# JGI-Bioinformatics/Kmernator

Hardware: AMD Instinct MI355X
Metric: total k-mers/sec at k=31, 150 bp reads (spectrum build, inputs resident in HBM) (higher is better)
Workload: dtype u64

## Files before the change

### kmernator_amd/csrc/kmr_api.hip

```cpp
#include <hip/hip_runtime.h>
#include <dlfcn.h>
#include <unistd.h>
#include <rccl/rccl.h>

#include <algorithm>
#include <atomic>
#include <cmath>
#include <cstdio>
#include <cstdlib>
#include <cstring>
#include <cctype>
#include <memory>
#include <string>
#include <type_traits>
#include <vector>

#include "../../include/kmernator_amd.h"
#include "kmr_kernels.hpp"
#include "kmr_partition.hpp"
#include "kmr_ingest.hpp"
#include "kmr_artifact.hpp"
#include "kmr_select.hpp"
#include "kmr_pairs.hpp"
#include "kmr_dump.hpp"
// ... 117 lines not shown
	uint64_t target_list = 2048;
	uint64_t sub_batch_bases = 0;
	int recycle = -1;
	int part_blocks = 0;
	double entry_share = -1.0;
	double early_entry_share = -1.0;
	uint64_t saturated_batch_bytes = 0;
	bool no_lut = false, no_narrow = false, no_l1_state = false, no_stream_lookups = false;
	uint64_t long_list_chunks = 0;
	uint64_t binned_min = 1ull << 18;
	uint64_t twobit_piece_bases = 0;
	uint64_t list_aim = 0;
	bool pow2_lists = false;
	bool no_packed_direct = false;
	bool no_uniform_count = false;
	bool no_lean_extract = false;
	bool exchange_fail_once = false;
	uint64_t dump_piece_bytes = 0;
	bool dump_timing = false;
	bool select_timing = false;
	bool pairs_timing = false;
	uint32_t pair_hash_bits = 64;
	bool no_coarse_lists = true;
};

struct kmr_handle : HandleMem, BuildMem, ExchangeMem {
	kmr_config cfg;
	Tuning tune;
	uint32_t k = 0, kb = 0, hkb = 0, W = 0;
	bool ext = false;
// ... 16 lines not shown
	long trk_next = 128; uint64_t trk_raw = 0, trk_good = 0; std::vector<unsigned long long> trk_bounds; std::vector<uint64_t> trk_snap_raw, trk_snap_good;
	bool sk_fast_div = false;
	bool sender_launch = false;
	bool sk_exchange = false;
	bool auto_mode = false;
	int bits1 = 0;
	uint64_t inserted_records = 0;
	uint64_t call_bases_hint = 0;
	uint32_t lut_log2 = 0;
	uint64_t lut_gen = ~0ull, map_gen = 0;
	hipStream_t tb_copy_stream = nullptr; hipEvent_t tb_ready[2] = {nullptr, nullptr}, tb_consumed[2] = {nullptr, nullptr}; bool tb_set_used[2] = {false, false};
	const SkPacked *packed_direct = nullptr;
	int uniform_q_hint = -1;
	uint32_t sk_bits = 0, sk_m = 0, sk_off = 0, sk_win = 0;
	double hP[256], hPk[256];
	uint32_t sk_uni_w = 0xffffffffu; bool sk_uni_mixed = false; bool last_count_uniform = false;
	uint32_t peer_uni_w = 0xffffffffu; bool peer_uni_mixed = false, peers_declare = false;
	uint64_t xr_lo = 0, xr_hi = ~0ull;
	uint64_t last_early_hi = 0, last_early_entries = 0;
	bool last_early_overflowed = false;
	double last_score_ms = 0, last_select_ms = 0, last_write_ms = 0;
	double last_dump_size_ms = 0, last_dump_write_ms = 0;
	double last_pairs_ms = 0, last_pairs_parse_ms = 0, last_pairs_sort_ms = 0;
	uint64_t last_pair_hash_collisions = 0;
	uint64_t last_saturated_keys = 0, last_saturated_batches = 0;
	bool qual_mixed = false;
	uint32_t sk_fine_shift = 0;
	uint32_t sk_min_override = 0;
	uint64_t xo_segcap = 0; std::vector<uint64_t> xo_counts; const void *xo_batch = nullptr; uint64_t xo_first = 0;
	void *xc_comm = nullptr; kmr_transport xc_tr = {nullptr, nullptr, nullptr};
	uint64_t xc_job_bases = 0, xc_bytes_to_peers = 0;
// ... 1435 lines not shown
		if (dv[1]) mixed = true;
		else if (dv[0] != SK_UNI_NONE) { if (w == SK_UNI_NONE) w = dv[0]; else if (w != dv[0]) mixed = true; }
	}
	if (!mixed && w != SK_UNI_NONE) { uni = true; uni_wbits = w; }
	return 0;
}
template <int W> SkLong<W> sk_own_lists(kmr_handle *h, bool refined) {
	SkLong<W> lg{};
	lg.list_first = 0; lg.list_stride = 1;
	if (h->sk_exchange && h->cfg.world_size > 1 && !refined) { lg.list_first = h->cfg.rank; lg.list_stride = h->cfg.world_size; }
	return lg;
}
template <int W> struct SkCountLaunch {
	void (*kern)(PoolView, const uint64_t *, const uint64_t *, uint64_t, uint32_t, CountOut, FinalizeParams, unsigned int *, uint32_t, SkTrackView, SkLong<W>);
	size_t smem;
};
template <int W, int LOG2S, bool TRACK, bool EXT, bool UNI> SkCountLaunch<W> sk_count_form() { return {sk_count_kernel<W, LOG2S, TRACK, EXT, UNI>, sk_count_smem_bytes<W, LOG2S, TRACK, EXT, UNI>()}; }
template <int W> int sk_count_select(kmr_handle *h, bool ext, bool tracking, bool uni, SkCountLaunch<W> &k) {
	k = ext ? sk_count_form<W, COUNT_LOG2S_EXT, false, true, false>() : (tracking ? sk_count_form<W, COUNT_LOG2S, true, false, false>() :
	    (uni ? sk_count_form<W, COUNT_LOG2S, false, false, true>() : sk_count_form<W, COUNT_LOG2S, false, false, false>()));
	const auto kern = k.kern; const size_t smem = k.smem;
	HIPCHK(h, hipFuncSetAttribute((const void *)kern, hipFuncAttributeMaxDynamicSharedMemorySize, (int)smem));
	return 0;
}

template <int W> struct SkFinalize {
	FinalizeParams f{}; bool keepSing = false, ext = false, tracking = false, refined = false, uni = false;
	uint64_t nl = 1; uint64_t *ls = nullptr, *lc = nullptr; uint32_t nch = 0;
	uint64_t wcap = 0, scap = 0, wmax = 0, smax = 0;
	uint32_t *wc = nullptr, *sc = nullptr; FinalizeCounters *fc = nullptr; unsigned long long *cursors = nullptr;
	SkTrackView tv{};
	SkLong<W> lgMain{}, lgItems{}; uint64_t n_items = 0;
	uint64_t early_slots = 0; FinalizeCounters early_c{};
	FinalizeCounters c{}; unsigned long long cur[2] = {0, 0};
};
// ... 123 lines not shown
		if (ext && (key_entries(h, h->uw_keys) < wcap || !h->uw_vals)) {
			h->uw_keys.reset(); h->uw_vals.reset();
			HIPCHK(h, h->uw_keys.alloc(8ull * W * wcap)); HIPCHK(h, h->uw_vals.alloc(4ull * vw * wcap));
		}
		if (key_entries(h, h->us_keys) < scap || !h->us_b8 || (ext && !h->us_pkt)) {
			h->us_keys.reset(); h->us_b8.reset(); h->us_pkt.reset();
			HIPCHK(h, h->us_keys.alloc(8ull * W * scap)); HIPCHK(h, h->us_b8.alloc(scap)); if (ext) HIPCHK(h, h->us_pkt.alloc(4 * scap));
		}
		HIPCHK(h, hipMemsetAsync(wc, 0, 4 * h->nb_weak, h->stream)); HIPCHK(h, hipMemsetAsync(sc, 0, 4 * h->nb_sing, h->stream));
		HIPCHK(h, hipMemsetAsync(fc, 0, sizeof(FinalizeCounters), h->stream)); HIPCHK(h, hipMemsetAsync(cursors, 0, 16, h->stream));
		const CountOut out = count_out(h, !ext, cursors, wc, sc, fc);
		rc = zero_work_counter(h); if (rc) return rc;
		const int grid = (int)std::min<uint64_t>((uint64_t)num_cus(h) * 4, (nl / p.lgMain.list_stride + SK_LBATCH) / SK_LBATCH);
		SkCountLaunch<W> k;
		rc = sk_count_select<W>(h, ext, tracking, p.uni, k); if (rc) return rc;
		if (tracking) HIPCHK(h, hipMemsetAsync(tv.d_unique, 0, 8 * (tv.n + 1), h->stream));
		if (dbg()) { int nb = 0; hipOccupancyMaxActiveBlocksPerMultiprocessor(&nb, (const void *)k.kern, SKC_THREADS, k.smem); fprintf(stderr, "sk_count<W=%d>: %d blocks per CU (LDS %zu), %llu lists, %u chunks\n", W, nb, k.smem, (unsigned long long)nl, p.nch); }
		hipLaunchKernelGGL(k.kern, dim3(grid), dim3(SKC_THREADS), k.smem, h->stream, pool_view(h, h->l1), p.ls, p.lc, nl, h->k, out, f, h->work_counter.get<unsigned int>(), sk_dbg_flags("KMR_SK_COUNT_DBG"), tv, p.lgMain);
		HIPCHK(h, hipGetLastError());
		DevBuf mslots, mext;
		if (n_items) {
			SkLong<W> &lgItems = p.lgItems;
			if (mslots.alloc(sizeof(Slot<W>) << merge_log2) != hipSuccess) return fail(h, KMR_ERR_OOM, "merge table of the long lists");
			if (ext && mext.alloc(sizeof(ExtSlot) << merge_log2) != hipSuccess) return fail(h, KMR_ERR_OOM, "merge table of the long lists");
			hipLaunchKernelGGL(table_clear_kernel<W>, dim3(grid_for(1ull << merge_log2)), dim3(256), 0, h->stream, mslots.get<Slot<W>>(), mext.get<ExtSlot>(), 1ull << merge_log2);
			lgItems.merge.slots = mslots.get<Slot<W>>(); lgItems.merge.ext = mext.get<ExtSlot>(); lgItems.merge.log2cap = merge_log2;
			HIPCHK(h, hipMemsetAsync(lgItems.merge_used, 0, 8, h->stream));
			rc = zero_work_counter(h); if (rc) return rc;
			const int grid2 = (int)std::min<uint64_t>((uint64_t)num_cus(h) * 4, n_items);
			hipLaunchKernelGGL(k.kern, dim3(grid2), dim3(SKC_THREADS), k.smem, h->stream, pool_view(h, h->l1), p.ls, p.lc, nl, h->k, out, f, h->work_counter.get<unsigned int>(), sk_dbg_flags("KMR_SK_COUNT_DBG"), tv, lgItems);
// ... 46 lines not shown
	p.keepSing = p.f.has_singletons && min_depth <= 1;
	p.ext = h->ext;
	p.tracking = h->cfg.size_tracker != 0;
	if (!h->l1.head) { rc = pool_reserve(h, h->l1, 0, false); if (rc) return rc; }
	rc = arena_reset(h); if (rc) return rc;
	p.nl = h->sk_state ? sk_list_count(h->sk_bits) : 1;
	if (h->sk_state) {
		hipLaunchKernelGGL(sk_close_kernel, dim3(grid_for(p.nl)), dim3(256), 0, h->stream, h->sk_state.get<unsigned long long>(), p.nl, h->l1.chunk_count.get<uint32_t>(), h->l1.cap);
		HIPCHK(h, hipGetLastError());
	}
	p.refined = h->sk_state && h->sk_fine_shift > 0;
	if (p.refined) { rc = sk_refine_lists(h, p.nl); if (rc) return rc; }
	rc = build_csr(h, h->l1, p.nl, 0, &p.ls, &p.lc, &p.nch); if (rc) return rc;
	rc = sk_entry_buffers<W>(h, p, h->stats.raw_good_kmers); if (rc) return rc;
	rc = sk_count_uniform<W>(h, p.tracking, p.uni, p.f.uni_wbits); if (rc) return rc;
	h->last_count_uniform = p.uni;
	if (p.tracking) { rc = sk_track_view(h, p.tv); if (rc) return rc; }
	p.lgMain = sk_own_lists<W>(h, p.refined);
	bool device_error = false;
	rc = sk_early_takeover<W>(h, p, min_depth, device_error); if (rc) return rc;
	if (device_error) { time_end(h, 1, ea, eb); return sync_state(h); }
	rc = sk_long_items<W>(h, p); if (rc) return rc;
	bool overflowed = false;
	rc = sk_count_pass<W>(h, p, overflowed); if (rc) return rc;
	if (overflowed) { time_end(h, 1, ea, eb); return fail(h, KMR_ERR_CAPACITY, "entry buffers of the count pass overflowed at their upper bound (internal sizing error)"); }
	h->stats.unique_kmers = p.c.unique;
	h->stats.singleton_kmers = p.f.has_singletons ? p.c.singletons : 0;
	if (p.tracking) { rc = sk_track_elements(h, p.tv, p.f.has_singletons); if (rc) return rc; }
	if (p.early_slots) { rc = sk_append_early<W>(h, p); if (rc) return rc; }
	h->early.active = false;
	hipEvent_t tma, tmb; time_begin(h, KMR_TIME_BUCKETS, &tma, &tmb);
// ... 238 lines not shown
int kmr_tune(kmr_handle *h, const char *knob, double value) {
	if (!h || !knob) return KMR_ERR_INVALID_ARG;
	const std::string k(knob);
	if (k == "target_list_records") h->tune.target_list = value >= 1 ? (uint64_t)value : 2048;
	else if (k == "sub_batch_bases") h->tune.sub_batch_bases = value >= 1 ? (uint64_t)value : 0;
	else if (k == "recycle_chunks") h->tune.recycle = value < 0 ? -1 : (value != 0 ? 1 : 0);
	else if (k == "partition_blocks") h->tune.part_blocks = value >= 1 ? (int)value : 0;
	else if (k == "entry_share") h->tune.entry_share = value;
	else if (k == "early_entry_share") h->tune.early_entry_share = value;
	else if (k == "saturated_batch_bytes") h->tune.saturated_batch_bytes = value >= 1 ? (uint64_t)value : 0;
	else if (k == "lookup_table") h->tune.no_lut = value == 0;
	else if (k == "stream_lookups") h->tune.no_stream_lookups = value == 0;
	else if (k == "long_list_chunks") h->tune.long_list_chunks = value < 2 ? 2 : (uint64_t)value;
	else if (k == "lean_extract") h->tune.no_lean_extract = value == 0;
	else if (k == "uniform_count") h->tune.no_uniform_count = value == 0;
	else if (k == "packed_direct") h->tune.no_packed_direct = value == 0;
	else if (k == "pow2_lists") h->tune.pow2_lists = value != 0;
	else if (k == "list_aim") h->tune.list_aim = value >= 1 ? (uint64_t)value : 0;
	else if (k == "twobit_piece_bases") h->tune.twobit_piece_bases = (uint64_t)value;
	else if (k == "exchange_fail_once") h->tune.exchange_fail_once = value != 0;
	else if (k == "binned_buckets_min") h->tune.binned_min = value >= 0 ? (uint64_t)value : ~0ull;
	else if (k == "coarse_lists") h->tune.no_coarse_lists = value == 0;
	else if (k == "select_timing") h->tune.select_timing = value != 0;
	else if (k == "dump_timing") h->tune.dump_timing = value != 0;
	else if (k == "pairs_timing") h->tune.pairs_timing = value != 0;
	else if (k == "pair_hash_bits") h->tune.pair_hash_bits = value >= 1 && value < 64 ? (uint32_t)value : 64;
	else if (k == "dump_piece_bytes") h->tune.dump_piece_bytes = value >= 1 ? (uint64_t)value : 0;
	else if (k == "narrow_tallies") h->tune.no_narrow = value == 0;
	else if (k == "keep_level1_state") h->tune.no_l1_state = value == 0;
	else if (k == "superkmer_window") {
		if (h->superkmer_mode && !h->sk_state) { uint32_t w, m, o; if (!sk_geometry(h->k, 0, w, m, o, (uint32_t)value)) return fail(h, KMR_ERR_INVALID_ARG, "no minimizer geometry under that window"); h->sk_win = w; h->sk_m = m; h->sk_off = o; }
	}
	else if (k == "superkmer_minimizer") {
		if (h->superkmer_mode && !h->sk_state) { uint32_t w, m, o; if (!sk_geometry(h->k, (uint32_t)value, w, m, o)) return fail(h, KMR_ERR_INVALID_ARG, "no minimizer geometry for that length"); h->sk_win = w; h->sk_m = m; h->sk_off = o; }
	}
	else return fail(h, KMR_ERR_INVALID_ARG, "unknown tuning knob '" + k + "'");
	return KMR_OK;
}

int kmr_build_info(kmr_handle *h, const char *what, double *value) {
	if (!h || !what || !value) return KMR_ERR_INVALID_ARG;
	const std::string k(what);
	if (k == "lists") *value = h->sk_state ? (double)sk_list_count(h->sk_bits) : 0.0;
	else if (k == "uniform_count") *value = h->last_count_uniform ? 1.0 : 0.0;
	else if (k == "chunk_pool_chunks") *value = (double)h->l1.cap;
	else if (k == "superkmer_window") *value = (double)h->sk_win;
	else if (k == "early_lists") *value = (double)h->last_early_hi;
	else if (k == "early_entries") *value = (double)h->last_early_entries;
	else if (k == "early_overflowed") *value = h->last_early_overflowed ? 1.0 : 0.0;
	else if (k == "saturated_keys") *value = (double)h->last_saturated_keys;
	else if (k == "saturated_batches") *value = (double)h->last_saturated_batches;
	else if (k == "device_blocks_live") *value = (double)g_blocks_live.load();
	else if (k == "filter_score_ms") *value = h->last_score_ms;
	else if (k == "select_ms") *value = h->last_select_ms;
	else if (k == "select_write_ms") *value = h->last_write_ms;
	else if (k == "pairs_ms") *value = h->last_pairs_ms;
	else if (k == "pairs_parse_ms") *value = h->last_pairs_parse_ms;
	else if (k == "pairs_sort_ms") *value = h->last_pairs_sort_ms;
	else if (k == "pair_hash_collisions") *value = (double)h->last_pair_hash_collisions;
// ... 1804 lines not shown
```

### kmernator_amd/csrc/kmr_instances.hpp

```cpp
#ifndef KMR_INSTANCES_HPP_
#define KMR_INSTANCES_HPP_

#include "kmr_superkmer.hpp"

namespace kmr {

static const int COUNT_LOG2S = 10;
static const int COUNT_LOG2S_EXT = 9;
static const int PD_THREADS = 1024, PD_RPT = 8, PD_LINE = 4;

#ifdef KMR_INSTANCES_EXTERN
#define KMR_T extern template
#else
#define KMR_T template
#endif

#define KMR_SKX(W, WIN, FILT) KMR_T __global__ void sk_extract_kernel<W, WIN, FILT, false>(ReadsView, DevParams, SkParams, PoolView); KMR_T __global__ void sk_extract_kernel<W, WIN, FILT, true>(ReadsView, DevParams, SkParams, PoolView);
#define KMR_SKXL(W, WIN) KMR_T __global__ void sk_extract_lean_kernel<W, WIN, false>(ReadsView, DevParams, SkParams, PoolView, float, SkPacked); KMR_T __global__ void sk_extract_lean_kernel<W, WIN, true>(ReadsView, DevParams, SkParams, PoolView, float, SkPacked);
#define KMR_SKX_W(W) KMR_SKX(W, 16, false) KMR_SKX(W, 16, true) KMR_SKX(W, 8, false) KMR_SKX(W, 8, true) KMR_SKX(W, 4, false) KMR_SKX(W, 4, true) KMR_SKXL(W, 16) KMR_SKXL(W, 8) KMR_SKXL(W, 4)

#define KMR_SKX_W32(W) KMR_SKX(W, 32, false) KMR_SKX(W, 32, true) KMR_SKXL(W, 32)

#define KMR_SKC(W, TRACK) KMR_SKCX(W, TRACK, false)
#define KMR_SKCX(W, TRACK, EXT) KMR_T __global__ void sk_count_kernel<W, EXT ? COUNT_LOG2S_EXT : COUNT_LOG2S, TRACK, EXT>(PoolView, const uint64_t *, const uint64_t *, uint64_t, uint32_t, CountOut, FinalizeParams, unsigned int *, uint32_t, SkTrackView, SkLong<W>);
#define KMR_SKL(W) KMR_T __global__ void sk_lookup_kernel<W>(PoolView, const uint64_t *, const uint64_t *, uint64_t, uint32_t, const uint64_t *, const uint64_t *, const uint32_t *, uint32_t *, uint64_t, unsigned int *, const uint64_t *, const uint64_t *, const uint32_t *, uint64_t, uint64_t);
#define KMR_SKCU(W) KMR_T __global__ void sk_count_kernel<W, COUNT_LOG2S, false, false, true>(PoolView, const uint64_t *, const uint64_t *, uint64_t, uint32_t, CountOut, FinalizeParams, unsigned int *, uint32_t, SkTrackView, SkLong<W>);
#define KMR_SKC_W(W) KMR_SKC(W, false) KMR_SKCU(W) KMR_SKC(W, true) KMR_SKCX(W, false, true) KMR_SKL(W)

#define KMR_EX(W, EXT, OP, SUB) KMR_T __global__ void extract_kernel<W, EXT, OP, SUB>(ReadsView, DevParams, OP);
#define KMR_EX_OP(W, EXT, ...) KMR_T __global__ void extract_kernel<W, EXT, __VA_ARGS__, false>(ReadsView, DevParams, __VA_ARGS__); KMR_T __global__ void extract_kernel<W, EXT, __VA_ARGS__, true>(ReadsView, DevParams, __VA_ARGS__);
#define KMR_EX_W(W) \
	KMR_EX_OP(W, false, InsertOp<W, false>) KMR_EX_OP(W, true, InsertOp<W, true>) \
	KMR_EX_OP(W, false, LinearOp<W, false, false>) KMR_EX_OP(W, false, LinearOp<W, false, true>) \
	KMR_EX_OP(W, true, LinearOp<W, true, false>) KMR_EX_OP(W, true, LinearOp<W, true, true>) \
	KMR_T __global__ void extract_kernel<W, false, LookupOp<W>, false>(ReadsView, DevParams, LookupOp<W>); \
	KMR_T __global__ void extract_kernel<W, false, LookupWeightOp<W>, false>(ReadsView, DevParams, LookupWeightOp<W>);

#define KMR_PD(W, EXT, LEVEL) KMR_T __global__ void partition_direct_kernel<W, EXT, LEVEL, PD_THREADS, PD_RPT, PD_LINE>(PartSource<W>, PoolView, unsigned int *, const int, const int);
#define KMR_OS(W, EXT, REQ) KMR_T __global__ void owner_scatter_kernel<W, EXT, REQ>(const typename PoolRec<W, EXT>::type *, const uint64_t *, const uint32_t *, uint64_t, uint32_t, uint32_t, uint32_t *, uint64_t, unsigned long long *, unsigned int *, uint32_t *, uint32_t *, OwnerFn);
#define KMR_CK(W, EXT, LOG2S, NARROW) KMR_T __global__ void count_kernel<W, EXT, LOG2S, NARROW>(PoolView, const uint64_t *, const uint64_t *, uint64_t, CountOut, FinalizeParams, unsigned int *, int);
#define KMR_PART_W(W) \
	KMR_PD(W, false, 1) KMR_PD(W, false, 2) KMR_PD(W, true, 1) KMR_PD(W, true, 2) \
	KMR_OS(W, false, false) KMR_OS(W, false, true) KMR_OS(W, true, false) KMR_OS(W, true, true) \
	KMR_CK(W, false, COUNT_LOG2S, false) KMR_CK(W, false, 11, false) KMR_CK(W, true, COUNT_LOG2S, false)

#if defined(KMR_INSTANCES_EXTERN)
KMR_SKX_W(1) KMR_SKX_W(2) KMR_SKX_W(3) KMR_SKX_W(4)
KMR_SKX_W32(2) KMR_SKX_W32(3) KMR_SKX_W32(4)
KMR_SKC_W(1) KMR_SKC_W(2) KMR_SKC_W(3) KMR_SKC_W(4)
KMR_EX_W(1) KMR_EX_W(2) KMR_EX_W(3) KMR_EX_W(4)
KMR_PART_W(1) KMR_PART_W(2) KMR_PART_W(3) KMR_PART_W(4)
KMR_CK(1, true, COUNT_LOG2S, true)
#else
#ifdef KMR_INST_SKX
KMR_SKX_W(KMR_INST_W)
#if KMR_INST_W > 1
KMR_SKX_W32(KMR_INST_W)
#endif
#endif
#ifdef KMR_INST_SKC
KMR_SKC_W(KMR_INST_W)
#endif
#ifdef KMR_INST_EX
KMR_EX_W(KMR_INST_W)
#endif
#ifdef KMR_INST_PART
KMR_PART_W(KMR_INST_W)
#if KMR_INST_W == 1
KMR_CK(1, true, COUNT_LOG2S, true)
#endif
#endif
#endif

}
#endif
```

### kmernator_amd/csrc/kmr_superkmer.hpp

```cpp
#ifndef KMR_SUPERKMER_HPP_
#define KMR_SUPERKMER_HPP_

#include "kmr_partition.hpp"
#include "kmr_buckets.hpp"

namespace kmr {

#ifndef KMR_SK_MAX_N
#define KMR_SK_MAX_N 128
#endif
static const uint32_t SK_CHUNK_G = 64;
static const uint32_t SK_MAX_N = KMR_SK_MAX_N;
static const int SK_WAVES = 3;
static const int SK_WINDOW = 16;
static const int SK_RR = 3, SKL_RR = 4;

#ifdef KMR_DEBUG_HOOKS
#define SK_DBG(flags, bit) (((flags) & (bit)) != 0)
#else
#define SK_DBG(flags, bit) false
#endif
struct SkTrackRec { uint32_t raw, good; unsigned long long end_ordinal; };
static const uint32_t SK_TRACK_MAX = 512;
struct SkTrackView { const unsigned long long *bounds; uint32_t n; unsigned int *d_unique, *d_single; };
// ... 1135 lines not shown

static const int SK_STAGE_CHUNKS = 4;
static const int SK_STAGE_G = SK_STAGE_CHUNKS * SK_CHUNK_G;
static const uint32_t SK_LBATCH = 24;
static const uint32_t SK_DESC_CAP = 160;

template <int W> struct SkLong {
	const uint64_t *item_c0, *item_c1;
	uint64_t n_items;
	uint64_t long_threshold;
	uint32_t list_first, list_stride;
	Table<W> merge;
	unsigned long long *merge_used;
};

template <int W, int LOG2S, bool TRACK = false, bool EXT = false, bool UNI = false>
__host__ __device__ constexpr size_t sk_count_smem_bytes() { return (size_t)(1 << LOG2S) * (8 * W + 24 + (W > 1 ? 4 : 0) - (UNI && W > 1 ? 12 : 0) + (TRACK ? 8 : 0) + (EXT ? 28 : 0)) + (size_t)SK_STAGE_G * 16 + 256 + 64 + (TRACK ? 8 * (SK_TRACK_MAX + 1) : 0); }
static const uint64_t SK_EXT_LONG_CHUNKS = 128;
static const int SK_EXT_BLOCKS = 3;
__device__ __forceinline__ uint32_t sk_ext_char(uint32_t code) { return (uint32_t)((0x584e54474341ull >> (8 * code)) & 0xffu); }

#ifndef KMR_SKC_WAVES
#define KMR_SKC_WAVES 4
#endif
static const int SKC_WAVES = KMR_SKC_WAVES, SKC_THREADS = SKC_WAVES * 64;
static const unsigned long long SK_KEY_PENDING = ~0ull;
static const uint32_t SK_ORDERED_FROM = 256;
static const unsigned long long SK_OSLAB = 2048;

template <int W, int LOG2S, bool TRACK = false, bool EXT = false, bool UNI = false>
__global__ __launch_bounds__(SKC_THREADS, EXT ? (W == 1 ? (LOG2S <= 9 ? SK_EXT_BLOCKS : 2) : 1) : ((W == 1 && LOG2S <= 10 && !TRACK) ? 4 : (W == 2 && LOG2S <= 10 && !TRACK ? (UNI ? 4 : 3) : 1)))
void sk_count_kernel(PoolView pool, const uint64_t *list_start, const uint64_t *list_chunks, uint64_t n_lists, uint32_t k,
                     CountOut out, FinalizeParams f, unsigned int *work_counter, uint32_t dbgFlags, SkTrackView tv, SkLong<W> lg) {
	static_assert(!UNI || (!TRACK && !EXT), "the one-weight count pass is the plain one's");
	constexpr int S = 1 << LOG2S;
	constexpr bool LEAN = UNI && W > 1;
#ifndef KMR_SKC_LIMIT_PCT
#define KMR_SKC_LIMIT_PCT 80
#endif
	constexpr uint32_t LIMIT = (uint32_t)(S * (KMR_SKC_LIMIT_PCT / 100.0));
	constexpr int WSLOTS = S / SKC_WAVES;
	extern __shared__ __attribute__((aligned(16))) uint8_t csm[];
	uint64_t *tkeys = (uint64_t *)csm;
	unsigned long long *tcnt = (unsigned long long *)(tkeys + (size_t)S * W);
	double *twsum = (double *)(tcnt + S);
	unsigned long long *tfirst = (unsigned long long *)(twsum + (LEAN ? 0 : S));
	uint32_t *tstate = (uint32_t *)(tfirst + S);
	uint32_t *ttally = tstate + (W > 1 && !LEAN ? S : 0);
	uint32_t *tpkt = ttally + (EXT ? 6 * S : 0);
	uint4 *stage = (uint4 *)(tpkt + (EXT ? S : 0));
	uint8_t *recOf = (uint8_t *)(stage + SK_STAGE_G);
	unsigned long long *tsecond = (unsigned long long *)(csm + (size_t)S * (8 * W + 24 + (W > 1 ? 4 : 0) + (EXT ? 28 : 0)) + (size_t)SK_STAGE_G * 16 + 256 + 64);
	unsigned int *trkU = (unsigned int *)(tsecond + (TRACK ? S : 0)), *trkS = trkU + (SK_TRACK_MAX + 1);
	__shared__ uint32_t s_list, s_sp;
	__shared__ uint32_t s_claimed[2], s_overflow[2];
	__shared__ uint32_t s_stackBits[40], s_stackVal[40];
	__shared__ unsigned long long s_c0[SK_LBATCH + 1], s_c1[SK_LBATCH + 1];
	__shared__ uint32_t s_dchunk[SK_DESC_CAP];
	__shared__ uint8_t s_dcount[SK_DESC_CAP];
	const int t = threadIdx.x, lane = t & 63, wv = t >> 6;
	if (TRACK) for (int i = t; i < 2 * (int)(SK_TRACK_MAX + 1); i += SKC_THREADS) trkU[i] = 0;
	const uint32_t vw = EXT ? 15 : 3;
	unsigned long long uniq = 0, single = 0, keptW = 0, keptS = 0, satK = 0, satS = 0;
	unsigned long long uniqW = 0, singleW = 0;
	unsigned long long wpos = 0, wend = 0, spos = 0, send = 0;
	bool outFull = false;
	if (t == 0) { s_claimed[0] = s_claimed[1] = 0; s_overflow[0] = s_overflow[1] = 0; s_sp = 0; }
	for (int i = t; i < S; i += SKC_THREADS) { tkeys[(size_t)i * W] = EMPTY_KEY; if (W > 1) tkeys[(size_t)i * W + W - 1] = SK_KEY_PENDING; tcnt[i] = 0; if constexpr (!LEAN) twsum[i] = 0.0; tfirst[i] = NO_FIRST; if constexpr (W > 1 && !LEAN) tstate[i] = 0; if (TRACK) tsecond[i] = NO_FIRST; }
	if (EXT) for (int i = t; i < 6 * S; i += SKC_THREADS) ttally[i] = 0;
	lds_barrier();
	const uint32_t singC = f.has_singletons ? (f.min_depth > 1 ? 0u : 2u) : 3u;
	const uint32_t weakMin = ((!f.has_singletons || f.min_depth > 2) && f.min_depth != 1) ? f.min_depth : 0u;
	const uint32_t uniFirst = UNI ? (first_weight_bits(__uint_as_float(f.uni_wbits)) & 0x7fffffu) : 0u;
	const uint4 *poolg = (const uint4 *)pool.base;
	uint4 pre = make_uint4(0, 0, 0, 0); uint32_t preCount = 0; uint64_t preList = ~0ull;
	uint32_t gen = 0;

	const bool itemMode = lg.item_c0 != nullptr;
	const uint32_t grab = itemMode ? 1u : SK_LBATCH;
	for (;;) {
		if (t == 0) s_list = atomicAdd(work_counter, grab);
		lds_barrier();
		const uint64_t lfirst = s_list;
// ... 19 lines not shown
		auto fetch = [&](uint64_t ci, uint4 &v, uint32_t &count) {
			uint32_t chunk;
			describe(ci, chunk, count);
			v = make_uint4(0, 0, 0, 0);
			if ((uint32_t)lane < count) v = poolg[(size_t)chunk * SK_CHUNK_G + lane];
		};
		for (uint32_t lj = 0; lj < nl; lj++) {
			const uint64_t c0 = s_c0[lj], c1 = s_c1[lj];
			if (c0 == c1) continue;
			if (itemMode && (__hip_atomic_load(out.err, __ATOMIC_RELAXED, __HIP_MEMORY_SCOPE_AGENT) & ERR_TABLE_FULL)) continue;
			uint32_t fl = gen & 1u;
			gen++;
			auto insert_pass = [&](const uint32_t bits, const uint32_t val, const bool firstPass) {
				const uint32_t subMask = bits ? ((1u << bits) - 1) : 0;
				const bool padded = W > 1 && (LEAN || (k & 31u) != 0);
				uint4 *wstage = stage + wv * SK_CHUNK_G;
				uint8_t *wrecOf = recOf + wv * 64;
				uint4 cur = make_uint4(0, 0, 0, 0); uint32_t curCount = 0;
				if (firstPass && preList == lfirst + lj) { cur = pre; curCount = preCount; }
				else if (c0 + wv < c1) fetch(c0 + wv, cur, curCount);
				bool wantPre = firstPass;
				if (firstPass) preList = ~0ull;
				for (uint64_t ci = c0 + wv; ci < c1 && !s_overflow[fl] && s_claimed[fl] <= LIMIT; ci += SKC_WAVES) {
					wstage[lane] = cur;
					const uint32_t glen = (cur.y >> 17) & 0x7fu;
					uint32_t claimedHere = 0;
					unsigned long long starts = 0;
					if (__all((lane & 1) != 0 || (uint32_t)lane >= curCount || glen == 2u)) starts = 0x5555555555555555ull & (curCount >= 64u ? ~0ull : ((1ull << curCount) - 1ull));
					else if (EXT && __all(((uint32_t)lane * 43u >> 7) * 3u != (uint32_t)lane || (uint32_t)lane >= curCount || glen == 3u)) starts = 0x9249249249249249ull & (curCount >= 64u ? ~0ull : ((1ull << curCount) - 1ull));
					else {
						const uint32_t hn = (cur.y >> 8) & 0xffu;
						const bool cand = (uint32_t)lane < curCount && hn >= 1u && hn <= SK_MAX_N && glen == sk_rec_granules(hn, k, ((cur.y >> 16) & 1u) != 0, EXT) && ((cur.y >> 30) & 1u) == (EXT ? 1u : 0u);
						const unsigned long long C = __ballot(cand), inRange = curCount >= 64u ? ~0ull : ((1ull << curCount) - 1ull);
						unsigned long long N = 0;
#pragma unroll
						for (uint32_t d = 2; d <= 9; d++) N |= __ballot(cand && glen == d) << d;
						if ((C & 1ull) && !__any(cand && glen > 9u) && (N & inRange) == (C & ~1ull)) starts = C;
						else for (uint32_t pos = 0; pos < curCount; ) {
						starts |= 1ull << pos;
						const uint32_t step = (uint32_t)__builtin_amdgcn_readlane((int)glen, (int)pos);
						pos += step ? step : SK_CHUNK_G;
					}
					}
					const bool isStart = (starts >> lane) & 1ull;
					const uint32_t myN = isStart ? (cur.y >> 8) & 0xffu : 0u;
					const uint32_t incl = sk_wave_scan_u32(myN);
					const uint32_t T = (uint32_t)__builtin_amdgcn_readlane((int)incl, 63);
					const uint32_t myOff = incl - myN;
					const uint32_t Lk = (T + 63u) >> 6;
					if (myN) {
						const float inv = __builtin_amdgcn_rcpf((float)Lk);
						const uint32_t l0 = (uint32_t)(((float)(myOff + Lk - 1) + 0.5f) * inv), l1 = (uint32_t)(((float)(myOff + myN - 1) + 0.5f) * inv);
						for (uint32_t l = l0; l <= l1 && l < 64u; l++) wrecOf[l] = (uint8_t)lane;
					}
					sk_wave_lds_order();
					const uint32_t e0 = (uint32_t)lane * Lk;
					uint32_t left = e0 < T ? (T - e0 < Lk ? T - e0 : Lk) : 0u;
					uint32_t rs = left ? wrecOf[lane] : 0u;
					uint32_t j = e0 - (uint32_t)__shfl((int)myOff, (int)rs, 64);
					uint32_t hx = (uint32_t)__shfl((int)cur.x, (int)rs, 64), hy = (uint32_t)__shfl((int)cur.y, (int)rs, 64), hw = (uint32_t)__shfl((int)cur.w, (int)rs, 64);
					if (SK_DBG(dbgFlags, 4)) left = 0;
					uint4 nxt = make_uint4(0, 0, 0, 0); uint32_t nxtCount = 0, nxtChunk = 0, preChunk = 0;
					const bool wantNxt = ci + SKC_WAVES < c1;
					bool havePre = false;
					if (wantNxt) describe(ci + SKC_WAVES, nxtChunk, nxtCount);
					if (wantPre) {
						wantPre = false;
						if (lj + 1 < nl) { const uint64_t n0 = s_c0[lj + 1], n1 = s_c1[lj + 1]; if (n0 + wv < n1) { describe(n0 + wv, preChunk, preCount); havePre = true; preList = lfirst + lj + 1; } }
					}
					if (wantNxt && (uint32_t)lane < nxtCount) nxt = poolg[(size_t)nxtChunk * SK_CHUNK_G + lane];
					if (havePre) { pre = make_uint4(0, 0, 0, 0); if ((uint32_t)lane < preCount) pre = poolg[(size_t)preChunk * SK_CHUNK_G + lane]; }
					uint32_t n = 0; const uint32_t *ww = nullptr; bool uniformW = true; uint64_t ord0 = 0;
					const uint8_t *xq = nullptr;
					uint32_t leftCarry = 0;
					auto enter_record = [&]() {
						n = (hy >> 8) & 0xffu;
						ww = (const uint32_t *)(wstage + rs + 1) + 4 * sk_base_granules(n, k);
						uniformW = ((hy >> 16) & 1u) != 0;
						ord0 = (uint64_t)hx | ((uint64_t)(hy & 0xffu) << 32);
						if (EXT) xq = (const uint8_t *)(ww + (uniformW ? 0u : 4u * ((n + 3) / 4)));
// ... 65 lines not shown
						if (EXT && j > 0) { const uint32_t b = j - 1; leftCarry = (((const uint32_t *)(wstage + rs + 1))[b >> 4] >> (30 - 2 * (b & 15u))) & 3u; }
						prepare(kA);
					}
					uint32_t dbgSink = 0;
					auto step_one = [&](KState &cur, KState &nxt) {
						if (left) {
							uint32_t s = cur.slot;
							const float wa = __uint_as_float(UNI ? f.uni_wbits : cur.w);
							unsigned long long old = EMPTY_KEY;
							const bool tableOn = !SK_DBG(dbgFlags, 1) && cur.mine;
							if (W == 1 || padded) { if (tableOn) old = atomicCAS((unsigned long long *)&tkeys[(size_t)s * W], (unsigned long long)EMPTY_KEY, (unsigned long long)cur.key.w[0]); }
							j++; left--; sb += 2;
							if (left) {
								if (j >= n) {
									rs = rs + ((hy >> 17) & 0x7fu);
									{ const uint32_t g0 = rs < SK_CHUNK_G - 1 ? rs : SK_CHUNK_G - 1; const uint4 hh = wstage[g0]; hx = hh.x; hy = hh.y; hw = hh.w; }
									j = 0;
									seed_window();
									enter_record();
								} else if (sb > 62u) seed_window();
								prepare(nxt);
							}
							if (SK_DBG(dbgFlags, 1)) { dbgSink ^= (uint32_t)cur.key.w[0] ^ s; }
							else if (cur.mine) {
								bool placed = false;
								const uint32_t claimedBefore = claimedHere;
								if constexpr (W == 1) {
									if (old == EMPTY_KEY) { claimedHere++; placed = true; }
									else if (old == cur.key.w[0]) placed = true;
									else s = (s + cur.step) & (S - 1);
								}
// ... 71 lines not shown
									}
								}
							}
						}
					};
					for (uint32_t it = 0; it < Lk; it += 2) { step_one(kA, kB); step_one(kB, kA); }
					if (SK_DBG(dbgFlags, 1) && dbgSink == 0x12345u) s_overflow[fl] = 2;
					claimedHere = (uint32_t)__builtin_amdgcn_readlane((int)sk_wave_scan_u32(claimedHere), 63);
					if (lane == 0 && claimedHere) atomicAdd(&s_claimed[fl], claimedHere);
					sk_wave_lds_order();
					cur = nxt; curCount = nxtCount;
				}
				if (wantPre && lj + 1 < nl) { const uint64_t n0 = s_c0[lj + 1], n1 = s_c1[lj + 1]; if (n0 + wv < n1) { fetch(n0 + wv, pre, preCount); preList = lfirst + lj + 1; } }
			};
			auto emit_pass = [&]() {
				uint16_t *wsel = (uint16_t *)(stage + wv * SK_CHUNK_G);
				static_assert(WSLOTS * 2 <= (int)SK_CHUNK_G * 16, "the selected slots' indices live in one staging quarter");
				uint32_t nsel = 0;
				unsigned long long usedMask[WSLOTS / 64];
				const unsigned long long below = (1ull << lane) - 1;
#pragma unroll
				for (int i = 0; i < WSLOTS / 64; i++) {
					const int s = wv * WSLOTS + i * 64 + lane;
					const uint32_t count = (uint32_t)tcnt[s];
					const bool used = count != 0;
					const unsigned long long um = __ballot(used);
					usedMask[i] = um;
					if (!itemMode) { uniqW += (uint32_t)__builtin_popcountll(um); singleW += (uint32_t)__builtin_popcountll(__ballot(count == 1)); }
					uint32_t cls = !used ? 0u : ((count == 1 && singC != 3u) ? singC : (count < weakMin ? 0u : 1u));
					if (SK_DBG(dbgFlags, 2)) cls = 0;
					const bool need = (itemMode || TRACK) ? used : cls != 0;
// ... 110 lines not shown
#pragma unroll
							for (int q = 0; q < W; q++) out.skeys[pos * W + q] = key.w[q];
							const float wf = (float)wsum;
							out.sweight[pos] = (uint8_t)((unsigned char)(((double)wf * 254.0)) + 1);
							if constexpr (EXT) out.spkt[pos] = tpkt[s];
						}
						bucket_count_add(out.singCount, bucket, cls == 2 && !outFull);
						if (!outFull) { spos += cnt; keptS += lane == 0 ? cnt : 0u; }
					}
				}
				sk_wave_lds_order();
#pragma unroll
				for (int i = 0; i < WSLOTS / 64; i++) {
					const int s = wv * WSLOTS + i * 64 + lane;
					if ((usedMask[i] >> lane) & 1ull) {
						tkeys[(size_t)s * W] = EMPTY_KEY; if (W > 1) tkeys[(size_t)s * W + W - 1] = SK_KEY_PENDING; tcnt[s] = 0; if constexpr (!LEAN) twsum[s] = 0.0; tfirst[s] = NO_FIRST; if constexpr (W > 1 && !LEAN) tstate[s] = 0; if (TRACK) tsecond[s] = NO_FIRST;
						if constexpr (EXT) {
#pragma unroll
							for (int q = 0; q < 6; q++) ttally[(size_t)s * 6 + q] = 0;
						}
					}
				}
			};
			auto clear_table = [&]() {
				for (int i = t; i < S; i += SKC_THREADS) { tkeys[(size_t)i * W] = EMPTY_KEY; if (W > 1) tkeys[(size_t)i * W + W - 1] = SK_KEY_PENDING; tcnt[i] = 0; if constexpr (!LEAN) twsum[i] = 0.0; tfirst[i] = NO_FIRST; if constexpr (W > 1 && !LEAN) tstate[i] = 0; if (TRACK) tsecond[i] = NO_FIRST; }
				if (EXT) for (int i = t; i < 6 * S; i += SKC_THREADS) ttally[i] = 0;
			};

			insert_pass(0, 0, true);
			lds_barrier();
			const bool ovf = s_overflow[fl] != 0 || s_claimed[fl] > LIMIT;
			if (t == 0) { s_claimed[fl ^ 1u] = 0; s_overflow[fl ^ 1u] = 0; }
			if (!ovf) {
				emit_pass();
				lds_barrier();
				continue;
			}
			clear_table();
			if (t == 0) { s_sp = 2; s_stackBits[0] = 1; s_stackVal[0] = 0; s_stackBits[1] = 1; s_stackVal[1] = 1; }
			lds_barrier();
// ... 664 lines not shown
```

Measured before the change: 55.86 billion.

## Process two chunks per wave iteration in the one-word uniform-weight count kernel

Adds a PAIR variant of the superkmer count kernel for W=1 with uniform weights. Each wave now stages and expands two pool chunks per loop step, packing both chunks' k-mer counts into one wave scan and distributing the combined work across lanes. The per-slot weight-sum array is dropped to make LDS room for the doubled staging area. This is meant to cut per-chunk loop overhead and lane underuse on short chunks, at the cost of more complex indexing and a second fetch per iteration.

```diff
diff --git a/kmernator_amd/csrc/kmr_api.hip b/kmernator_amd/csrc/kmr_api.hip
--- a/kmernator_amd/csrc/kmr_api.hip
+++ b/kmernator_amd/csrc/kmr_api.hip
@@ -155,6 +155,7 @@
 	bool pow2_lists = false;
 	bool no_packed_direct = false;
 	bool no_uniform_count = false;
+	bool no_pair_chunks = false;
 	bool no_lean_extract = false;
 	bool exchange_fail_once = false;
 	uint64_t dump_piece_bytes = 0;
@@ -201,7 +202,7 @@
 	int uniform_q_hint = -1;
 	uint32_t sk_bits = 0, sk_m = 0, sk_off = 0, sk_win = 0;
 	double hP[256], hPk[256];
-	uint32_t sk_uni_w = 0xffffffffu; bool sk_uni_mixed = false; bool last_count_uniform = false;
+	uint32_t sk_uni_w = 0xffffffffu; bool sk_uni_mixed = false; bool last_count_uniform = false, last_count_pair = false;
 	uint32_t peer_uni_w = 0xffffffffu; bool peer_uni_mixed = false, peers_declare = false;
 	uint64_t xr_lo = 0, xr_hi = ~0ull;
 	uint64_t last_early_hi = 0, last_early_entries = 0;
@@ -1667,11 +1668,13 @@
 template <int W> struct SkCountLaunch {
 	void (*kern)(PoolView, const uint64_t *, const uint64_t *, uint64_t, uint32_t, CountOut, FinalizeParams, unsigned int *, uint32_t, SkTrackView, SkLong<W>);
 	size_t smem;
+	bool pair;
 };
-template <int W, int LOG2S, bool TRACK, bool EXT, bool UNI> SkCountLaunch<W> sk_count_form() { return {sk_count_kernel<W, LOG2S, TRACK, EXT, UNI>, sk_count_smem_bytes<W, LOG2S, TRACK, EXT, UNI>()}; }
+template <int W, int LOG2S, bool TRACK, bool EXT, bool UNI, bool PAIR = false> SkCountLaunch<W> sk_count_form() { return {sk_count_kernel<W, LOG2S, TRACK, EXT, UNI, PAIR>, sk_count_smem_bytes<W, LOG2S, TRACK, EXT, UNI, PAIR>(), PAIR}; }
 template <int W> int sk_count_select(kmr_handle *h, bool ext, bool tracking, bool uni, SkCountLaunch<W> &k) {
 	k = ext ? sk_count_form<W, COUNT_LOG2S_EXT, false, true, false>() : (tracking ? sk_count_form<W, COUNT_LOG2S, true, false, false>() :
 	    (uni ? sk_count_form<W, COUNT_LOG2S, false, false, true>() : sk_count_form<W, COUNT_LOG2S, false, false, false>()));
+	if constexpr (W == 1) { if (uni && !ext && !tracking && !h->tune.no_pair_chunks) k = sk_count_form<1, COUNT_LOG2S, false, false, true, true>(); }
 	const auto kern = k.kern; const size_t smem = k.smem;
 	HIPCHK(h, hipFuncSetAttribute((const void *)kern, hipFuncAttributeMaxDynamicSharedMemorySize, (int)smem));
 	return 0;
@@ -1825,6 +1828,7 @@
 		const int grid = (int)std::min<uint64_t>((uint64_t)num_cus(h) * 4, (nl / p.lgMain.list_stride + SK_LBATCH) / SK_LBATCH);
 		SkCountLaunch<W> k;
 		rc = sk_count_select<W>(h, ext, tracking, p.uni, k); if (rc) return rc;
+		h->last_count_pair = k.pair;
 		if (tracking) HIPCHK(h, hipMemsetAsync(tv.d_unique, 0, 8 * (tv.n + 1), h->stream));
 		if (dbg()) { int nb = 0; hipOccupancyMaxActiveBlocksPerMultiprocessor(&nb, (const void *)k.kern, SKC_THREADS, k.smem); fprintf(stderr, "sk_count<W=%d>: %d blocks per CU (LDS %zu), %llu lists, %u chunks\n", W, nb, k.smem, (unsigned long long)nl, p.nch); }
 		hipLaunchKernelGGL(k.kern, dim3(grid), dim3(SKC_THREADS), k.smem, h->stream, pool_view(h, h->l1), p.ls, p.lc, nl, h->k, out, f, h->work_counter.get<unsigned int>(), sk_dbg_flags("KMR_SK_COUNT_DBG"), tv, p.lgMain);
@@ -1901,7 +1905,7 @@
 	rc = build_csr(h, h->l1, p.nl, 0, &p.ls, &p.lc, &p.nch); if (rc) return rc;
 	rc = sk_entry_buffers<W>(h, p, h->stats.raw_good_kmers); if (rc) return rc;
 	rc = sk_count_uniform<W>(h, p.tracking, p.uni, p.f.uni_wbits); if (rc) return rc;
-	h->last_count_uniform = p.uni;
+	h->last_count_uniform = p.uni; h->last_count_pair = false;
 	if (p.tracking) { rc = sk_track_view(h, p.tv); if (rc) return rc; }
 	p.lgMain = sk_own_lists<W>(h, p.refined);
 	bool device_error = false;
@@ -2170,6 +2174,7 @@
 	else if (k == "long_list_chunks") h->tune.long_list_chunks = value < 2 ? 2 : (uint64_t)value;
 	else if (k == "lean_extract") h->tune.no_lean_extract = value == 0;
 	else if (k == "uniform_count") h->tune.no_uniform_count = value == 0;
+	else if (k == "pair_chunks") h->tune.no_pair_chunks = value == 0;
 	else if (k == "packed_direct") h->tune.no_packed_direct = value == 0;
 	else if (k == "pow2_lists") h->tune.pow2_lists = value != 0;
 	else if (k == "list_aim") h->tune.list_aim = value >= 1 ? (uint64_t)value : 0;
@@ -2199,6 +2204,7 @@
 	const std::string k(what);
 	if (k == "lists") *value = h->sk_state ? (double)sk_list_count(h->sk_bits) : 0.0;
 	else if (k == "uniform_count") *value = h->last_count_uniform ? 1.0 : 0.0;
+	else if (k == "pair_chunks") *value = h->last_count_pair ? 1.0 : 0.0;
 	else if (k == "chunk_pool_chunks") *value = (double)h->l1.cap;
 	else if (k == "superkmer_window") *value = (double)h->sk_win;
 	else if (k == "early_lists") *value = (double)h->last_early_hi;
diff --git a/kmernator_amd/csrc/kmr_instances.hpp b/kmernator_amd/csrc/kmr_instances.hpp
--- a/kmernator_amd/csrc/kmr_instances.hpp
+++ b/kmernator_amd/csrc/kmr_instances.hpp
@@ -26,6 +26,7 @@
 #define KMR_SKL(W) KMR_T __global__ void sk_lookup_kernel<W>(PoolView, const uint64_t *, const uint64_t *, uint64_t, uint32_t, const uint64_t *, const uint64_t *, const uint32_t *, uint32_t *, uint64_t, unsigned int *, const uint64_t *, const uint64_t *, const uint32_t *, uint64_t, uint64_t);
 #define KMR_SKCU(W) KMR_T __global__ void sk_count_kernel<W, COUNT_LOG2S, false, false, true>(PoolView, const uint64_t *, const uint64_t *, uint64_t, uint32_t, CountOut, FinalizeParams, unsigned int *, uint32_t, SkTrackView, SkLong<W>);
 #define KMR_SKC_W(W) KMR_SKC(W, false) KMR_SKCU(W) KMR_SKC(W, true) KMR_SKCX(W, false, true) KMR_SKL(W)
+#define KMR_SKCP KMR_T __global__ void sk_count_kernel<1, COUNT_LOG2S, false, false, true, true>(PoolView, const uint64_t *, const uint64_t *, uint64_t, uint32_t, CountOut, FinalizeParams, unsigned int *, uint32_t, SkTrackView, SkLong<1>);
 
 #define KMR_EX(W, EXT, OP, SUB) KMR_T __global__ void extract_kernel<W, EXT, OP, SUB>(ReadsView, DevParams, OP);
 #define KMR_EX_OP(W, EXT, ...) KMR_T __global__ void extract_kernel<W, EXT, __VA_ARGS__, false>(ReadsView, DevParams, __VA_ARGS__); KMR_T __global__ void extract_kernel<W, EXT, __VA_ARGS__, true>(ReadsView, DevParams, __VA_ARGS__);
@@ -47,7 +48,7 @@
 #if defined(KMR_INSTANCES_EXTERN)
 KMR_SKX_W(1) KMR_SKX_W(2) KMR_SKX_W(3) KMR_SKX_W(4)
 KMR_SKX_W32(2) KMR_SKX_W32(3) KMR_SKX_W32(4)
-KMR_SKC_W(1) KMR_SKC_W(2) KMR_SKC_W(3) KMR_SKC_W(4)
+KMR_SKC_W(1) KMR_SKC_W(2) KMR_SKC_W(3) KMR_SKC_W(4) KMR_SKCP
 KMR_EX_W(1) KMR_EX_W(2) KMR_EX_W(3) KMR_EX_W(4)
 KMR_PART_W(1) KMR_PART_W(2) KMR_PART_W(3) KMR_PART_W(4)
 KMR_CK(1, true, COUNT_LOG2S, true)
@@ -60,6 +61,9 @@
 #endif
 #ifdef KMR_INST_SKC
 KMR_SKC_W(KMR_INST_W)
+#if KMR_INST_W == 1
+KMR_SKCP
+#endif
 #endif
 #ifdef KMR_INST_EX
 KMR_EX_W(KMR_INST_W)
diff --git a/kmernator_amd/csrc/kmr_superkmer.hpp b/kmernator_amd/csrc/kmr_superkmer.hpp
--- a/kmernator_amd/csrc/kmr_superkmer.hpp
+++ b/kmernator_amd/csrc/kmr_superkmer.hpp
@@ -1173,8 +1173,8 @@
 	unsigned long long *merge_used;
 };
 
-template <int W, int LOG2S, bool TRACK = false, bool EXT = false, bool UNI = false>
-__host__ __device__ constexpr size_t sk_count_smem_bytes() { return (size_t)(1 << LOG2S) * (8 * W + 24 + (W > 1 ? 4 : 0) - (UNI && W > 1 ? 12 : 0) + (TRACK ? 8 : 0) + (EXT ? 28 : 0)) + (size_t)SK_STAGE_G * 16 + 256 + 64 + (TRACK ? 8 * (SK_TRACK_MAX + 1) : 0); }
+template <int W, int LOG2S, bool TRACK = false, bool EXT = false, bool UNI = false, bool PAIR = false>
+__host__ __device__ constexpr size_t sk_count_smem_bytes() { return (size_t)(1 << LOG2S) * (8 * W + 24 + (W > 1 ? 4 : 0) - (UNI && W > 1 ? 12 : 0) - (PAIR ? 8 : 0) + (TRACK ? 8 : 0) + (EXT ? 28 : 0)) + (size_t)SK_STAGE_G * 16 * (PAIR ? 2 : 1) + 256 + 64 + (TRACK ? 8 * (SK_TRACK_MAX + 1) : 0); }
 static const uint64_t SK_EXT_LONG_CHUNKS = 128;
 static const int SK_EXT_BLOCKS = 3;
 __device__ __forceinline__ uint32_t sk_ext_char(uint32_t code) { return (uint32_t)((0x584e54474341ull >> (8 * code)) & 0xffu); }
@@ -1187,13 +1187,16 @@
 static const uint32_t SK_ORDERED_FROM = 256;
 static const unsigned long long SK_OSLAB = 2048;
 
-template <int W, int LOG2S, bool TRACK = false, bool EXT = false, bool UNI = false>
+template <int W, int LOG2S, bool TRACK = false, bool EXT = false, bool UNI = false, bool PAIR = false>
 __global__ __launch_bounds__(SKC_THREADS, EXT ? (W == 1 ? (LOG2S <= 9 ? SK_EXT_BLOCKS : 2) : 1) : ((W == 1 && LOG2S <= 10 && !TRACK) ? 4 : (W == 2 && LOG2S <= 10 && !TRACK ? (UNI ? 4 : 3) : 1)))
 void sk_count_kernel(PoolView pool, const uint64_t *list_start, const uint64_t *list_chunks, uint64_t n_lists, uint32_t k,
                      CountOut out, FinalizeParams f, unsigned int *work_counter, uint32_t dbgFlags, SkTrackView tv, SkLong<W> lg) {
 	static_assert(!UNI || (!TRACK && !EXT), "the one-weight count pass is the plain one's");
+	static_assert(!PAIR || (UNI && W == 1), "chunk pairs: one-word keys in the one-weight form (its staging lies where the weight sums were)");
 	constexpr int S = 1 << LOG2S;
 	constexpr bool LEAN = UNI && W > 1;
+	constexpr bool NOWSUM = LEAN || PAIR;
+	constexpr uint32_t NH = PAIR ? 2 : 1, WG = NH * SK_CHUNK_G;
 #ifndef KMR_SKC_LIMIT_PCT
 #define KMR_SKC_LIMIT_PCT 80
 #endif
@@ -1203,12 +1206,12 @@
 	uint64_t *tkeys = (uint64_t *)csm;
 	unsigned long long *tcnt = (unsigned long long *)(tkeys + (size_t)S * W);
 	double *twsum = (double *)(tcnt + S);
-	unsigned long long *tfirst = (unsigned long long *)(twsum + (LEAN ? 0 : S));
+	unsigned long long *tfirst = (unsigned long long *)(twsum + (NOWSUM ? 0 : S));
 	uint32_t *tstate = (uint32_t *)(tfirst + S);
 	uint32_t *ttally = tstate + (W > 1 && !LEAN ? S : 0);
 	uint32_t *tpkt = ttally + (EXT ? 6 * S : 0);
 	uint4 *stage = (uint4 *)(tpkt + (EXT ? S : 0));
-	uint8_t *recOf = (uint8_t *)(stage + SK_STAGE_G);
+	uint8_t *recOf = (uint8_t *)(stage + SK_STAGE_G * NH);
 	unsigned long long *tsecond = (unsigned long long *)(csm + (size_t)S * (8 * W + 24 + (W > 1 ? 4 : 0) + (EXT ? 28 : 0)) + (size_t)SK_STAGE_G * 16 + 256 + 64);
 	unsigned int *trkU = (unsigned int *)(tsecond + (TRACK ? S : 0)), *trkS = trkU + (SK_TRACK_MAX + 1);
 	__shared__ uint32_t s_list, s_sp;
@@ -1225,7 +1228,7 @@
 	unsigned long long wpos = 0, wend = 0, spos = 0, send = 0;
 	bool outFull = false;
 	if (t == 0) { s_claimed[0] = s_claimed[1] = 0; s_overflow[0] = s_overflow[1] = 0; s_sp = 0; }
-	for (int i = t; i < S; i += SKC_THREADS) { tkeys[(size_t)i * W] = EMPTY_KEY; if (W > 1) tkeys[(size_t)i * W + W - 1] = SK_KEY_PENDING; tcnt[i] = 0; if constexpr (!LEAN) twsum[i] = 0.0; tfirst[i] = NO_FIRST; if constexpr (W > 1 && !LEAN) tstate[i] = 0; if (TRACK) tsecond[i] = NO_FIRST; }
+	for (int i = t; i < S; i += SKC_THREADS) { tkeys[(size_t)i * W] = EMPTY_KEY; if (W > 1) tkeys[(size_t)i * W + W - 1] = SK_KEY_PENDING; tcnt[i] = 0; if constexpr (!NOWSUM) twsum[i] = 0.0; tfirst[i] = NO_FIRST; if constexpr (W > 1 && !LEAN) tstate[i] = 0; if (TRACK) tsecond[i] = NO_FIRST; }
 	if (EXT) for (int i = t; i < 6 * S; i += SKC_THREADS) ttally[i] = 0;
 	lds_barrier();
 	const uint32_t singC = f.has_singletons ? (f.min_depth > 1 ? 0u : 2u) : 3u;
@@ -1275,17 +1278,15 @@
 			auto insert_pass = [&](const uint32_t bits, const uint32_t val, const bool firstPass) {
 				const uint32_t subMask = bits ? ((1u << bits) - 1) : 0;
 				const bool padded = W > 1 && (LEAN || (k & 31u) != 0);
-				uint4 *wstage = stage + wv * SK_CHUNK_G;
+				uint4 *wstage = stage + wv * WG;
 				uint8_t *wrecOf = recOf + wv * 64;
 				uint4 cur = make_uint4(0, 0, 0, 0); uint32_t curCount = 0;
 				if (firstPass && preList == lfirst + lj) { cur = pre; curCount = preCount; }
 				else if (c0 + wv < c1) fetch(c0 + wv, cur, curCount);
 				bool wantPre = firstPass;
 				if (firstPass) preList = ~0ull;
-				for (uint64_t ci = c0 + wv; ci < c1 && !s_overflow[fl] && s_claimed[fl] <= LIMIT; ci += SKC_WAVES) {
-					wstage[lane] = cur;
+				auto record_starts = [&](const uint4 &cur, const uint32_t curCount) -> unsigned long long {
 					const uint32_t glen = (cur.y >> 17) & 0x7fu;
-					uint32_t claimedHere = 0;
 					unsigned long long starts = 0;
 					if (__all((lane & 1) != 0 || (uint32_t)lane >= curCount || glen == 2u)) starts = 0x5555555555555555ull & (curCount >= 64u ? ~0ull : ((1ull << curCount) - 1ull));
 					else if (EXT && __all(((uint32_t)lane * 43u >> 7) * 3u != (uint32_t)lane || (uint32_t)lane >= curCount || glen == 3u)) starts = 0x9249249249249249ull & (curCount >= 64u ? ~0ull : ((1ull << curCount) - 1ull));
@@ -1303,28 +1304,52 @@
 						pos += step ? step : SK_CHUNK_G;
 					}
 					}
+					return starts;
+				};
+				for (uint64_t ci = c0 + wv; ci < c1 && !s_overflow[fl] && s_claimed[fl] <= LIMIT; ci += SKC_WAVES * NH) {
+					uint4 cur2 = make_uint4(0, 0, 0, 0); uint32_t cur2Count = 0;
+					if constexpr (PAIR) { if (ci + SKC_WAVES < c1) fetch(ci + SKC_WAVES, cur2, cur2Count); }
+					wstage[lane] = cur;
+					uint32_t claimedHere = 0;
+					const unsigned long long starts = record_starts(cur, curCount);
 					const bool isStart = (starts >> lane) & 1ull;
 					const uint32_t myN = isStart ? (cur.y >> 8) & 0xffu : 0u;
-					const uint32_t incl = sk_wave_scan_u32(myN);
-					const uint32_t T = (uint32_t)__builtin_amdgcn_readlane((int)incl, 63);
-					const uint32_t myOff = incl - myN;
+					uint32_t myN2 = 0;
+					if constexpr (PAIR) {
+						wstage[SK_CHUNK_G + lane] = cur2;
+						const unsigned long long starts2 = record_starts(cur2, cur2Count);
+						myN2 = ((starts2 >> lane) & 1ull) ? (cur2.y >> 8) & 0xffu : 0u;
+					}
+					const uint32_t incl = sk_wave_scan_u32(PAIR ? (myN | (myN2 << 16)) : myN);
+					const uint32_t tot = (uint32_t)__builtin_amdgcn_readlane((int)incl, 63);
+					const uint32_t T1 = PAIR ? (tot & 0xffffu) : tot, T = PAIR ? T1 + (tot >> 16) : tot;
+					const uint32_t myOff = (PAIR ? (incl & 0xffffu) : incl) - myN, myOff2 = PAIR ? T1 + (incl >> 16) - myN2 : 0u;
 					const uint32_t Lk = (T + 63u) >> 6;
-					if (myN) {
+					auto tell_lanes = [&](const uint32_t off, const uint32_t n, const uint32_t g) {
 						const float inv = __builtin_amdgcn_rcpf((float)Lk);
-						const uint32_t l0 = (uint32_t)(((float)(myOff + Lk - 1) + 0.5f) * inv), l1 = (uint32_t)(((float)(myOff + myN - 1) + 0.5f) * inv);
-						for (uint32_t l = l0; l <= l1 && l < 64u; l++) wrecOf[l] = (uint8_t)lane;
-					}
+						const uint32_t l0 = (uint32_t)(((float)(off + Lk - 1) + 0.5f) * inv), l1 = (uint32_t)(((float)(off + n - 1) + 0.5f) * inv);
+						for (uint32_t l = l0; l <= l1 && l < 64u; l++) wrecOf[l] = (uint8_t)g;
+					};
+					if (myN) tell_lanes(myOff, myN, (uint32_t)lane);
+					if constexpr (PAIR) { if (myN2) tell_lanes(myOff2, myN2, SK_CHUNK_G + (uint32_t)lane); }
 					sk_wave_lds_order();
 					const uint32_t e0 = (uint32_t)lane * Lk;
 					uint32_t left = e0 < T ? (T - e0 < Lk ? T - e0 : Lk) : 0u;
 					uint32_t rs = left ? wrecOf[lane] : 0u;
-					uint32_t j = e0 - (uint32_t)__shfl((int)myOff, (int)rs, 64);
-					uint32_t hx = (uint32_t)__shfl((int)cur.x, (int)rs, 64), hy = (uint32_t)__shfl((int)cur.y, (int)rs, 64), hw = (uint32_t)__shfl((int)cur.w, (int)rs, 64);
+					uint32_t j, hx, hy, hw;
+					if constexpr (PAIR) {
+						const uint32_t offs = (uint32_t)__shfl((int)(myOff | (myOff2 << 16)), (int)(rs & 63u), 64);
+						j = e0 - (rs >= SK_CHUNK_G ? offs >> 16 : offs & 0xffffu);
+						const uint4 hh = wstage[rs]; hx = hh.x; hy = hh.y; hw = hh.w;
+					} else {
+						j = e0 - (uint32_t)__shfl((int)myOff, (int)rs, 64);
+						hx = (uint32_t)__shfl((int)cur.x, (int)rs, 64); hy = (uint32_t)__shfl((int)cur.y, (int)rs, 64); hw = (uint32_t)__shfl((int)cur.w, (int)rs, 64);
+					}
 					if (SK_DBG(dbgFlags, 4)) left = 0;
 					uint4 nxt = make_uint4(0, 0, 0, 0); uint32_t nxtCount = 0, nxtChunk = 0, preChunk = 0;
-					const bool wantNxt = ci + SKC_WAVES < c1;
+					const bool wantNxt = ci + SKC_WAVES * NH < c1;
 					bool havePre = false;
-					if (wantNxt) describe(ci + SKC_WAVES, nxtChunk, nxtCount);
+					if (wantNxt) describe(ci + SKC_WAVES * NH, nxtChunk, nxtCount);
 					if (wantPre) {
 						wantPre = false;
 						if (lj + 1 < nl) { const uint64_t n0 = s_c0[lj + 1], n1 = s_c1[lj + 1]; if (n0 + wv < n1) { describe(n0 + wv, preChunk, preCount); havePre = true; preList = lfirst + lj + 1; } }
@@ -1420,7 +1445,8 @@
 							if (left) {
 								if (j >= n) {
 									rs = rs + ((hy >> 17) & 0x7fu);
-									{ const uint32_t g0 = rs < SK_CHUNK_G - 1 ? rs : SK_CHUNK_G - 1; const uint4 hh = wstage[g0]; hx = hh.x; hy = hh.y; hw = hh.w; }
+									if constexpr (PAIR) { if (rs >= curCount && rs < SK_CHUNK_G) rs = SK_CHUNK_G; }
+									{ const uint32_t g0 = rs < WG - 1 ? rs : WG - 1; const uint4 hh = wstage[g0]; hx = hh.x; hy = hh.y; hw = hh.w; }
 									j = 0;
 									seed_window();
 									enter_record();
@@ -1522,7 +1548,7 @@
 				if (wantPre && lj + 1 < nl) { const uint64_t n0 = s_c0[lj + 1], n1 = s_c1[lj + 1]; if (n0 + wv < n1) { fetch(n0 + wv, pre, preCount); preList = lfirst + lj + 1; } }
 			};
 			auto emit_pass = [&]() {
-				uint16_t *wsel = (uint16_t *)(stage + wv * SK_CHUNK_G);
+				uint16_t *wsel = (uint16_t *)(stage + wv * WG);
 				static_assert(WSLOTS * 2 <= (int)SK_CHUNK_G * 16, "the selected slots' indices live in one staging quarter");
 				uint32_t nsel = 0;
 				unsigned long long usedMask[WSLOTS / 64];
@@ -1663,7 +1689,7 @@
 				for (int i = 0; i < WSLOTS / 64; i++) {
 					const int s = wv * WSLOTS + i * 64 + lane;
 					if ((usedMask[i] >> lane) & 1ull) {
-						tkeys[(size_t)s * W] = EMPTY_KEY; if (W > 1) tkeys[(size_t)s * W + W - 1] = SK_KEY_PENDING; tcnt[s] = 0; if constexpr (!LEAN) twsum[s] = 0.0; tfirst[s] = NO_FIRST; if constexpr (W > 1 && !LEAN) tstate[s] = 0; if (TRACK) tsecond[s] = NO_FIRST;
+						tkeys[(size_t)s * W] = EMPTY_KEY; if (W > 1) tkeys[(size_t)s * W + W - 1] = SK_KEY_PENDING; tcnt[s] = 0; if constexpr (!NOWSUM) twsum[s] = 0.0; tfirst[s] = NO_FIRST; if constexpr (W > 1 && !LEAN) tstate[s] = 0; if (TRACK) tsecond[s] = NO_FIRST;
 						if constexpr (EXT) {
 #pragma unroll
 							for (int q = 0; q < 6; q++) ttally[(size_t)s * 6 + q] = 0;
@@ -1672,7 +1698,7 @@
 				}
 			};
 			auto clear_table = [&]() {
-				for (int i = t; i < S; i += SKC_THREADS) { tkeys[(size_t)i * W] = EMPTY_KEY; if (W > 1) tkeys[(size_t)i * W + W - 1] = SK_KEY_PENDING; tcnt[i] = 0; if constexpr (!LEAN) twsum[i] = 0.0; tfirst[i] = NO_FIRST; if constexpr (W > 1 && !LEAN) tstate[i] = 0; if (TRACK) tsecond[i] = NO_FIRST; }
+				for (int i = t; i < S; i += SKC_THREADS) { tkeys[(size_t)i * W] = EMPTY_KEY; if (W > 1) tkeys[(size_t)i * W + W - 1] = SK_KEY_PENDING; tcnt[i] = 0; if constexpr (!NOWSUM) twsum[i] = 0.0; tfirst[i] = NO_FIRST; if constexpr (W > 1 && !LEAN) tstate[i] = 0; if (TRACK) tsecond[i] = NO_FIRST; }
 				if (EXT) for (int i = t; i < 6 * S; i += SKC_THREADS) ttally[i] = 0;
 			};
 
```

Result: no change. 56.34 billion, median of 6 (+0.9%).
